# DefaultRui/VLN-VER

Measured on AMD Instinct MI355X. Metric: viewpoints/sec (multi-view->voxel fwd+bwd), vocc.py config, higher is better.
Workload: dtype bf16

## Files before the change

include/ver_ops.h:

```cpp
#ifndef VER_OPS_H
#define VER_OPS_H

#include <stdint.h>

#ifdef __cplusplus
extern "C" {
#endif

#define VER_ABI_VERSION 31

#define VER_OK            0
#define VER_EINVAL       -1
#define VER_EUNSUPPORTED -2
#define VER_ELAUNCH      -3

#define VER_F32  0
#define VER_BF16 1

int         ver_abi_version(void);
const char* ver_last_error(void);

int ver_msda_forward(const float* value, const int64_t* shapes_hw, const int64_t* level_start,
                     const float* loc, const float* attn_w, float* out,
                     int B, int num_keys, int heads, int head_dim, int levels, int points,
// ... 25 lines not shown

int ver_hits_from_mask(const uint8_t* bev_mask, int B, int Ncam, int Nq, int D,
                       uint8_t* vis, int32_t* vis_list, int32_t* vis_cnt,
                       int32_t* zero_list, int32_t* zero_cnt, int32_t* fwd_list, int32_t* fwd_cnt,
                       void* stream);

#define VER_SCA_ROWS_PREZEROED 1
#define VER_SCA_VALUE_HEAD_MAJOR 2
#define VER_SCA_GRAD_SLOTS_BF16 4
int ver_sca_head_major_supported(int value_dtype, int head_dim, int points, int map_h, int map_w);
int ver_sca_zero_rows(const int32_t* zero_list, const int32_t* zero_cnt, float* slots, int B, int Nq, int row_floats,
                      void* stream);
int ver_sca_forward(const void* value, int value_dtype, const float* offsets, const float* logits,
                    const float* uv, const uint8_t* vis, const int32_t* vis_list,
                    const int32_t* vis_cnt, const int32_t* zero_list, const int32_t* zero_cnt,
                    const int32_t* fwd_list, const int32_t* fwd_cnt,
                    float* slots,
                    int B, int Ncam, int Nq, int D, int heads, int head_dim, int points,
                    int map_h, int map_w, int flags, void* stream);

int ver_sca_backward_grad_dtype(int value_dtype, int head_dim, int points, int map_h, int map_w);
int ver_sca_backward(const void* value, int value_dtype, const float* offsets, const float* logits,
                     const float* uv, const uint8_t* vis, const int32_t* vis_list,
                     const int32_t* vis_cnt, const int32_t* fwd_list, const int32_t* fwd_cnt,
                     const void* grad_slots,
                     void* grad_value, int grad_value_dtype, float* grad_offsets, float* grad_logits,
                     int B, int Ncam, int Nq, int D, int heads, int head_dim, int points,
                     int map_h, int map_w, int flags, void* stream);

int ver_lattice_im2col(const void* src, void* col, const int* taps, int ntaps,
                       int B, int Z, int H, int W, int C, int dtype, void* stream);
int ver_lattice_col2im(const void* grad_col, void* grad_src, const int* taps, int ntaps,
                       int B, int Z, int H, int W, int C, int dtype, void* stream);

int ver_lattice_gather(const void* src, void* col, const int* taps, const long* col_offset, long col_stride,
                       int ntaps, int B, int Zr, int Zs, int H, int W, int C, int layout, int dtype,
                       const void* const_rows, const long* const_offset, int const_blocks, int const_width, void* stream);
int ver_lattice_scatter(const void* grad_col, void* grad_src, const int* taps, const long* col_offset,
                        long col_stride, int ntaps, int B, int Zr, int Zs, int H, int W, int C, int layout, int dtype,
                        void* stream);

int ver_convt_weight_forward(const float* weight, void* taps, long pairs, int dtype, void* stream);
int ver_convt_weight_backward(const void* grad_taps, float* grad_weight, long pairs, int dtype, void* stream);
int ver_convt_weight_backward_blocks(const void* blocks, const long* block_offsets, long ld, const void* prev_bias,
                                     const void* grad_v, float* grad_weight, int ci, int co, int dtype, void* stream);
int ver_convt_weight_forward_blocks(const float* weight, const long* block_offsets, long ld, void* blocks, int ci, int co,
                                    int dtype, void* stream);
int ver_blocks_vec_forward(const void* blocks, const long* block_rows, int nblocks, long ld, int ci, int ncols, const float* x,
                           float* vec, int dtype, void* stream);
int ver_blocks_vec_backward(const void* blocks, const long* block_rows, int nblocks, long ld, int ci, int ncols,
                            const float* grad_vec, float* grad_x, int dtype, void* stream);
int ver_lattice_transpose(void* channels_last, void* channel_first, long cf_stride, int B, int Z, int H, int W,
                          int C, int layout, int to_channel_first, int dtype, void* stream);
int ver_lattice_rows(void* channels_last, void* rows, long quarter, int period, int nseg, const int* seg_off,
                     const int* seg_len, const long* seg_base, const int* seg_pitch, const int* seg_rows, int B, int Z,
                     int H, int W, int C, int layout, int to_rows, int dtype, void* stream);

int ver_ln_relu_forward(const void* x, const float* gamma, const float* beta, void* y,
                        float* mean, float* rstd, long N, int W, float eps, int dtype, void* stream);
int ver_ln_relu_backward(const void* x, const void* grad_y, const float* gamma, const float* beta,
                         const float* mean, const float* rstd, void* grad_x,
                         float* grad_gamma, float* grad_beta, long N, int W, int dtype, void* stream);

int ver_focal_loss_blocks(long N, int C);
int ver_focal_loss_forward(const void* logits, const int64_t* target, float* partial, long N, int C,
                           float gamma, float alpha, int dtype, int32_t* bad_labels, void* stream);
int ver_focal_loss_forward_grad(const void* logits, const int64_t* target, float* partial, void* grad, long N, int C,
                                float gamma, float alpha, int dtype, int32_t* bad_labels, void* stream);
int ver_focal_loss_forward_grad_u8(const void* logits, const uint8_t* target, float* partial, void* grad, long N, int C,
                                   float gamma, float alpha, int dtype, int32_t* bad_labels, void* stream);
int ver_focal_loss_backward(const void* logits, const int64_t* target, const float* scale, void* grad,
                            long N, int C, float gamma, float alpha, int dtype, void* stream);

int ver_add_ln_forward(const void* a, int a_dtype, const float* residual, const float* gamma, const float* beta,
                       const int64_t* seed, float p_drop, float eps, float* y, void* y_bf16, float* mean,
                       float* rstd, long N, int C, void* stream);
int ver_add_ln_backward(const float* grad_y, const void* grad_y_bf16, const void* a, int a_dtype,
                        const float* residual, const float* gamma, const float* mean, const float* rstd,
                        const int64_t* seed, float p_drop, void* grad_a, float* grad_residual, float* grad_gamma,
                        float* grad_beta, long N, int C, void* stream);
int ver_relu_dropout_forward(const void* x, void* y, const int64_t* seed, float p_drop, long n, int dtype, void* stream);
int ver_relu_dropout_backward(const void* y, const void* grad_y, void* grad_x, float p_drop, long n, int dtype,
                              void* stream);

int ver_run_gather(const void* image, long image_stride, const int32_t* run_start, const int32_t* aug_idx,
                   void* rows, int B, int n_rows, int runs, int run_len, int n_aug, int row_elems, int dtype,
                   void* stream);
int ver_run_scatter(const void* rows, void* image, long image_stride, const int32_t* run_start, int B,
                    int n_rows, int runs, int run_len, int row_elems, int dtype, void* stream);

#define VER_OCC_MLP_CENTERED 2
long ver_occ_mlp_image_bytes(void);
int ver_occ_mlp_vector_floats(void);
int ver_occ_mlp_pack(const float* W1, const float* W2, const float* W3, void* image, void* stream);
int ver_occ_mlp_forward(const void* x, const void* image, const float* vectors, void* logits,
                        long N, int width, int classes, float eps, int first_linear, void* stream);
int ver_occ_mlp_forward_stats(const void* x, const void* image, const float* vectors, void* logits, float* rstd,
                              long N, int width, int classes, float eps, int first_linear, void* stream);
int ver_occ_mlp_backward(const void* x, const void* grad_logits, const void* image, const float* vectors,
                         void* grad_x, void* grad_a1, void* grad_a2, void* h1,
                         float* param_grads, long N, int width, int classes, float eps, int first_linear,
                         void* stream);
int ver_occ_mlp_backward_fused(const void* x, const void* grad_logits, const float* W2, const float* W3,
                               const float* vectors, void* grad_x, float* param_grads, long N, int width,
                               int classes, float eps, const float* grad_scale, int flags, void* stream);
int ver_occ_mlp_backward_fused_stats(const void* x, const void* grad_logits, const float* W2, const float* W3,
                                     const float* vectors, const float* rstd, void* grad_x, float* param_grads, long N,
                                     int width, int classes, float eps, const float* grad_scale, int flags, void* stream);

long ver_occ_predict_blocks(long N);
int  ver_occ_predict(const void* logits, int dtype, long N, int C, float threshold, int32_t* block_work,
                     int64_t* pairs, int64_t* count, void* stream);

int  ver_occ_confusion(const void* logits, int dtype, long rows_per_sample, int samples, int C, const uint8_t* labels,
                       const float* thresholds, int num_thresholds, int64_t* hist, void* stream);

int  ver_wgrad_tn_splits(long M, int Ka, int N);
int  ver_wgrad_tn_splits_ld(long M, int Ka, int N, long ld);
long ver_wgrad_tn_workspace(long M, int Ka, int N, int splits);
int  ver_wgrad_tn(const void* a, long lda, const void* g, long ldg, long M, int Ka, int N, void* out, long ldo,
                  int out_dtype, int splits, int flags, void* workspace, long workspace_bytes, void* stream);
int  ver_wgrad_tn_segments(const void* lattice, int layout, int B, int H, int W, int C, const int* taps, int nseg, const void* cst,
                           int ncst, int cw, const void* g, long ldg, int N, void* out, long ldo, int out_dtype, int splits,
                           void* workspace, long workspace_bytes, void* stream);
int  ver_wgrad_tn_segments_splits(int B, int H, int W, long Ka, int N, long ldg);

int  ver_gemm_nn(const void* a, long lda, const void* w, long ldw, const float* bias, void* c, long ldc, long M, int K,
                 int N, int flags, void* stream);
int  ver_gemm_nn_taps(const void* lattice, int layout, int B, int H, int W, int C, const int* taps, int ntaps, const void* w,
                      long ldw, const float* rowpos, const float* bias, void* c, long ldc, int N, void* stream);
int  ver_gemm_nn_segments(const void* lattice, int layout, int B, int H, int W, int C, const int* taps, int ntaps,
                          const void* cst, int ncst, int cw, const void* w, long ldw, const float* rowpos, const float* bias,
                          void* c, long ldc, int N, void* stream);
int  ver_gemm_nn_planes(const void* lattice, int layout, int B, int H, int W, int C, long plane_elems, int nplanes,
                        const int* tap_plane, const int* taps, int ntaps, const void* cst, int ncst, int cw, const void* w,
                        long ldw, const float* rowpos, const float* bias, void* c, long ldc, int N, void* stream);
int  ver_gemm_nn_splits(long M, int K, int N);
int  ver_gemm_nn_splitk(const void* a, long lda, const void* w, long ldw, const float* bias, void* c, long ldc, long M, int K,
                        int N, int splits, void* workspace, long workspace_bytes, void* stream);

int ver_clip_adamw_step(void* const* table, const long* sizes, const int* chunk_tensor, const int* chunk_index,
                        int n_tensors, int n_chunks, int chunk_elems, float* partial, float* norm_out, float max_norm,
                        float lr, float beta1, float beta2, float eps, float weight_decay, long step, void* stream);

int ver_clip_adamw_step_tensors(void* const* table, const long* sizes, const int* chunk_tensor, const int* chunk_index,
                                const float* hyper, int* steps, int n_tensors, int n_chunks, int chunk_elems, float* partial,
                                float* norm_out, float max_norm, void* stream);

int ver_lsa_solve(const float* cost, const int32_t* ncols, int32_t* match, int32_t* bad,
                  int P, int R, int Ccap, void* stream);

#ifdef __cplusplus
}
#endif
#endif
```

vln-ver_amd/csrc/ver_addln.hip:

```cpp
#include "ver_common.h"

namespace {
constexpr int kMaxK = 4;

__device__ __forceinline__ uint32_t f2bf(float f) {
    const uint32_t u = __float_as_uint(f);
    if ((u & 0x7fffffffu) > 0x7f800000u) return (u >> 16) | 0x40u;
    return (u + 0x7fffu + ((u >> 16) & 1u)) >> 16;
}

__device__ __forceinline__ bool keep_elem(uint64_t idx, uint64_t seed, uint32_t thresh) {
    uint64_t h = idx * 0x9E3779B97F4A7C15ull + seed;
    h ^= h >> 33;
    h *= 0xff51afd7ed558ccdull;
    h ^= h >> 33;
    h *= 0xc4ceb9fe1a85ec53ull;
    h ^= h >> 33;
    return (uint32_t)(h & 0xffffffu) < thresh;
}

template <bool ABF16>
__device__ __forceinline__ void load_a4(const void* a, long off, float (&v)[4]) {
    if (ABF16) {
        const uint2 t = *reinterpret_cast<const uint2*>(reinterpret_cast<const uint16_t*>(a) + off);
        v[0] = __uint_as_float(t.x << 16);
        v[1] = __uint_as_float(t.x & 0xffff0000u);
        v[2] = __uint_as_float(t.y << 16);
        v[3] = __uint_as_float(t.y & 0xffff0000u);
    } else {
        const float4 t = *reinterpret_cast<const float4*>(reinterpret_cast<const float*>(a) + off);
        v[0] = t.x; v[1] = t.y; v[2] = t.z; v[3] = t.w;
    }
}

__device__ __forceinline__ void store_bf4(uint16_t* p, long off, const float (&v)[4]) {
    uint2 t;
    t.x = f2bf(v[0]) | (f2bf(v[1]) << 16);
    t.y = f2bf(v[2]) | (f2bf(v[3]) << 16);
    *reinterpret_cast<uint2*>(p + off) = t;
}

template <bool ABF16, int K>
__device__ __forceinline__ void load_x(const void* a, const float* res, long row, int C, int lane, bool drop,
                                       uint64_t seed, uint32_t thresh, float scale, float (&x)[K][4],
                                       bool (&keep)[K][4]) {
#pragma unroll
    for (int k = 0; k < K; ++k) {
        const long off = row * C + 4 * (lane + 64 * k);
        float av[4];
        load_a4<ABF16>(a, off, av);
        const float4 r = *reinterpret_cast<const float4*>(res + off);
        const float rv[4] = {r.x, r.y, r.z, r.w};
#pragma unroll
        for (int i = 0; i < 4; ++i) {
            keep[k][i] = !drop || keep_elem((uint64_t)(off + i), seed, thresh);
            x[k][i] = rv[i] + (keep[k][i] ? av[i] * scale : 0.0f);
        }
    }
}
}

template <bool ABF16, int K>
__global__ __launch_bounds__(256) void k_add_ln_fwd(const void* __restrict__ a, const float* __restrict__ res,
                                                    const float* __restrict__ gamma, const float* __restrict__ beta,
                                                    const int64_t* __restrict__ seed_p, float p_drop, float eps,
                                                    float* __restrict__ y, uint16_t* __restrict__ y16,
                                                    float* __restrict__ mean, float* __restrict__ rstd, long N) {
    constexpr int C = 256 * K;
    const int lane = threadIdx.x & 63, wave = threadIdx.x >> 6;
    const bool drop = p_drop > 0.0f;
    const uint64_t seed = drop ? (uint64_t)seed_p[0] : 0ull;
    const uint32_t thresh = (uint32_t)((1.0f - p_drop) * 16777216.0f);
    const float scale = drop ? 1.0f / (1.0f - p_drop) : 1.0f;
    float g[K][4], bt[K][4];
#pragma unroll
    for (int k = 0; k < K; ++k) {
        const float4 gv = *reinterpret_cast<const float4*>(gamma + 4 * (lane + 64 * k));
        const float4 bv = *reinterpret_cast<const float4*>(beta + 4 * (lane + 64 * k));
        g[k][0] = gv.x; g[k][1] = gv.y; g[k][2] = gv.z; g[k][3] = gv.w;
        bt[k][0] = bv.x; bt[k][1] = bv.y; bt[k][2] = bv.z; bt[k][3] = bv.w;
    }
    for (long row = (long)blockIdx.x * 4 + wave; row < N; row += (long)gridDim.x * 4) {
        float x[K][4];
        bool keep[K][4];
        load_x<ABF16, K>(a, res, row, C, lane, drop, seed, thresh, scale, x, keep);
        float s = 0.0f;
#pragma unroll
        for (int k = 0; k < K; ++k) s += (x[k][0] + x[k][1]) + (x[k][2] + x[k][3]);
        const float mu = group_sum<64>(s) * (1.0f / C);
        float q = 0.0f;
#pragma unroll
        for (int k = 0; k < K; ++k)
#pragma unroll
            for (int i = 0; i < 4; ++i) {
                x[k][i] -= mu;
                q += x[k][i] * x[k][i];
            }
        const float rs = rsqrtf(group_sum<64>(q) * (1.0f / C) + eps);
        if (lane == 0) {
            mean[row] = mu;
            rstd[row] = rs;
        }
#pragma unroll
        for (int k = 0; k < K; ++k) {
            const long off = row * C + 4 * (lane + 64 * k);
            float o[4];
#pragma unroll
            for (int i = 0; i < 4; ++i) o[i] = x[k][i] * rs * g[k][i] + bt[k][i];
            *reinterpret_cast<float4*>(y + off) = make_float4(o[0], o[1], o[2], o[3]);
            if (y16) store_bf4(y16, off, o);
        }
    }
}

template <bool ABF16, int K>
__global__ __launch_bounds__(256) void k_add_ln_bwd(const float* __restrict__ dy, const uint16_t* __restrict__ dy16,
                                                    const void* __restrict__ a, const float* __restrict__ res,
                                                    const float* __restrict__ gamma, const float* __restrict__ mean,
                                                    const float* __restrict__ rstd, const int64_t* __restrict__ seed_p,
                                                    float p_drop, void* __restrict__ d_a, float* __restrict__ d_res,
                                                    float* __restrict__ dgamma, float* __restrict__ dbeta, long N) {
    constexpr int C = 256 * K;
    __shared__ float red[2][4][C];
    const int lane = threadIdx.x & 63, wave = threadIdx.x >> 6;
    const bool drop = p_drop > 0.0f;
    const uint64_t seed = drop ? (uint64_t)seed_p[0] : 0ull;
    const uint32_t thresh = (uint32_t)((1.0f - p_drop) * 16777216.0f);
    const float scale = drop ? 1.0f / (1.0f - p_drop) : 1.0f;
    float g[K][4], dg[K][4], db[K][4];
#pragma unroll
    for (int k = 0; k < K; ++k) {
        const float4 gv = *reinterpret_cast<const float4*>(gamma + 4 * (lane + 64 * k));
        g[k][0] = gv.x; g[k][1] = gv.y; g[k][2] = gv.z; g[k][3] = gv.w;
#pragma unroll
        for (int i = 0; i < 4; ++i) dg[k][i] = db[k][i] = 0.0f;
    }
    for (long row = (long)blockIdx.x * 4 + wave; row < N; row += (long)gridDim.x * 4) {
        float x[K][4], go[K][4];
        bool keep[K][4];
        load_x<ABF16, K>(a, res, row, C, lane, drop, seed, thresh, scale, x, keep);
        const float mu = mean[row], rs = rstd[row];
        float s1 = 0.0f, s2 = 0.0f;
#pragma unroll
        for (int k = 0; k < K; ++k) {
            const long off = row * C + 4 * (lane + 64 * k);
            const float4 t = *reinterpret_cast<const float4*>(dy + off);
            go[k][0] = t.x; go[k][1] = t.y; go[k][2] = t.z; go[k][3] = t.w;
            if (dy16) {
                float h[4];
                load_a4<true>(dy16, off, h);
#pragma unroll
                for (int i = 0; i < 4; ++i) go[k][i] += h[i];
            }
#pragma unroll
            for (int i = 0; i < 4; ++i) {
                x[k][i] = (x[k][i] - mu) * rs;
                dg[k][i] += go[k][i] * x[k][i];
                db[k][i] += go[k][i];
                go[k][i] *= g[k][i];
                s1 += go[k][i];
                s2 += go[k][i] * x[k][i];
            }
        }
        const float m1 = group_sum<64>(s1) * (1.0f / C), m2 = group_sum<64>(s2) * (1.0f / C);
#pragma unroll
        for (int k = 0; k < K; ++k) {
            const long off = row * C + 4 * (lane + 64 * k);
            float dx[4], da[4];
#pragma unroll
            for (int i = 0; i < 4; ++i) {
                dx[i] = (go[k][i] - m1 - x[k][i] * m2) * rs;
                da[i] = keep[k][i] ? dx[i] * scale : 0.0f;
            }
            *reinterpret_cast<float4*>(d_res + off) = make_float4(dx[0], dx[1], dx[2], dx[3]);
            if (ABF16)
                store_bf4(reinterpret_cast<uint16_t*>(d_a), off, da);
            else
                *reinterpret_cast<float4*>(reinterpret_cast<float*>(d_a) + off) = make_float4(da[0], da[1], da[2], da[3]);
        }
    }
#pragma unroll
    for (int k = 0; k < K; ++k)
#pragma unroll
        for (int i = 0; i < 4; ++i) {
            red[0][wave][4 * (lane + 64 * k) + i] = dg[k][i];
            red[1][wave][4 * (lane + 64 * k) + i] = db[k][i];
        }
    __syncthreads();
    for (int e = threadIdx.x; e < C; e += 256) {
        atomicAdd(dgamma + e, (red[0][0][e] + red[0][1][e]) + (red[0][2][e] + red[0][3][e]));
        atomicAdd(dbeta + e, (red[1][0][e] + red[1][1][e]) + (red[1][2][e] + red[1][3][e]));
    }
}

namespace {
int check_add_ln(const char* who, const void* a, const float* res, const float* gamma, long N, int C, int a_dtype,
                 float p_drop, const int64_t* seed) {
    VER_REQUIRE(N >= 0, VER_EINVAL, "%s: negative row count", who);
    VER_REQUIRE(C > 0 && C % 256 == 0 && C <= 256 * kMaxK, VER_EUNSUPPORTED,
                "%s: built for rows of 256, 512, 768 or 1024 channels (got %d)", who, C);
    VER_REQUIRE(a_dtype == VER_F32 || a_dtype == VER_BF16, VER_EINVAL, "%s: dtype %d is neither VER_F32 nor VER_BF16", who,
                a_dtype);
    VER_REQUIRE(p_drop >= 0.0f && p_drop < 1.0f, VER_EINVAL, "%s: dropout probability %g outside [0, 1)", who, p_drop);
    if (N == 0) return VER_OK;
    VER_REQUIRE(a && res && gamma && (seed || p_drop == 0.0f), VER_EINVAL, "%s: null pointer argument", who);
    VER_REQUIRE(((uintptr_t)a & 15) == 0 && ((uintptr_t)res & 15) == 0, VER_EINVAL, "%s: buffers must be 16-byte aligned", who);
    return VER_OK;
}
}

extern "C" int ver_add_ln_forward(const void* a, int a_dtype, const float* residual, const float* gamma,
                                  const float* beta, const int64_t* seed, float p_drop, float eps, float* y,
                                  void* y_bf16, float* mean, float* rstd, long N, int C, void* stream) {
    int rc = check_add_ln("ver_add_ln_forward", a, residual, gamma, N, C, a_dtype, p_drop, seed);
    if (rc) return rc;
    if (N == 0) return VER_OK;
    VER_REQUIRE(beta && y && mean && rstd, VER_EINVAL, "ver_add_ln_forward: null pointer argument");
    const unsigned grid = (unsigned)(((N + 3) / 4) < 8192 ? ((N + 3) / 4) : 8192);
    hipStream_t st = (hipStream_t)stream;
#define VER_FWD(BF, K_)                                                                                          \
    hipLaunchKernelGGL((k_add_ln_fwd<BF, K_>), dim3(grid), dim3(256), 0, st, a, residual, gamma, beta, seed, p_drop, \
                       eps, y, (uint16_t*)y_bf16, mean, rstd, N)
#define VER_FWD_K(BF)                        \
    do {                                     \
        if (C == 256) VER_FWD(BF, 1);        \
        else if (C == 512) VER_FWD(BF, 2);   \
        else if (C == 768) VER_FWD(BF, 3);   \
        else VER_FWD(BF, 4);                 \
    } while (0)
    if (a_dtype == VER_BF16) VER_FWD_K(true); else VER_FWD_K(false);
#undef VER_FWD_K
#undef VER_FWD
    return ver_check_launch("ver_add_ln_forward");
}

extern "C" int ver_add_ln_backward(const float* grad_y, const void* grad_y_bf16, const void* a, int a_dtype,
                                   const float* residual, const float* gamma, const float* mean, const float* rstd,
                                   const int64_t* seed, float p_drop, void* grad_a, float* grad_residual,
                                   float* grad_gamma, float* grad_beta, long N, int C, void* stream) {
    int rc = check_add_ln("ver_add_ln_backward", a, residual, gamma, N, C, a_dtype, p_drop, seed);
    if (rc) return rc;
    VER_REQUIRE(grad_gamma && grad_beta, VER_EINVAL, "ver_add_ln_backward: null parameter-gradient pointer");
    hipStream_t st = (hipStream_t)stream;
    int zrc = ver_zero_async(grad_gamma, C * sizeof(float), st);
    if (!zrc) zrc = ver_zero_async(grad_beta, C * sizeof(float), st);
    if (zrc) return zrc;
    hipError_t e = hipSuccess;
    if (e != hipSuccess) return ver_fail(VER_ELAUNCH, "ver_add_ln_backward: memset: %s", hipGetErrorString(e));
    if (N == 0) return VER_OK;
    VER_REQUIRE(grad_y && mean && rstd && grad_a && grad_residual, VER_EINVAL, "ver_add_ln_backward: null pointer argument");
    const unsigned grid = (unsigned)(((N + 3) / 4) < 2048 ? ((N + 3) / 4) : 2048);
#define VER_BWD(BF, K_)                                                                                           \
    hipLaunchKernelGGL((k_add_ln_bwd<BF, K_>), dim3(grid), dim3(256), 0, st, grad_y, (const uint16_t*)grad_y_bf16, a, \
                       residual, gamma, mean, rstd, seed, p_drop, grad_a, grad_residual, grad_gamma, grad_beta, N)
#define VER_BWD_K(BF)                        \
    do {                                     \
        if (C == 256) VER_BWD(BF, 1);        \
        else if (C == 512) VER_BWD(BF, 2);   \
        else if (C == 768) VER_BWD(BF, 3);   \
        else VER_BWD(BF, 4);                 \
    } while (0)
    if (a_dtype == VER_BF16) VER_BWD_K(true); else VER_BWD_K(false);
#undef VER_BWD_K
#undef VER_BWD
    return ver_check_launch("ver_add_ln_backward");
}

template <bool BF16>
__global__ __launch_bounds__(256) void k_relu_dropout_fwd(const void* __restrict__ x, void* __restrict__ y,
                                                          const int64_t* __restrict__ seed_p, float p_drop, long n4) {
    const bool drop = p_drop > 0.0f;
    const uint64_t seed = drop ? (uint64_t)seed_p[0] : 0ull;
    const uint32_t thresh = (uint32_t)((1.0f - p_drop) * 16777216.0f);
    const float scale = drop ? 1.0f / (1.0f - p_drop) : 1.0f;
    for (long i = (long)blockIdx.x * 256 + threadIdx.x; i < n4; i += (long)gridDim.x * 256) {
        float v[4];
        load_a4<BF16>(x, 4 * i, v);
#pragma unroll
        for (int j = 0; j < 4; ++j)
            v[j] = (v[j] > 0.0f && (!drop || keep_elem((uint64_t)(4 * i + j), seed, thresh))) ? v[j] * scale : 0.0f;
        if (BF16)
            store_bf4(reinterpret_cast<uint16_t*>(y), 4 * i, v);
        else
            *reinterpret_cast<float4*>(reinterpret_cast<float*>(y) + 4 * i) = make_float4(v[0], v[1], v[2], v[3]);
    }
}

template <bool BF16>
__global__ __launch_bounds__(256) void k_relu_dropout_bwd(const void* __restrict__ y, const void* __restrict__ dy,
                                                          void* __restrict__ dx, float scale, long n4) {
    for (long i = (long)blockIdx.x * 256 + threadIdx.x; i < n4; i += (long)gridDim.x * 256) {
        float v[4], g[4];
        load_a4<BF16>(y, 4 * i, v);
        load_a4<BF16>(dy, 4 * i, g);
#pragma unroll
        for (int j = 0; j < 4; ++j) g[j] = v[j] > 0.0f ? g[j] * scale : 0.0f;
        if (BF16)
            store_bf4(reinterpret_cast<uint16_t*>(dx), 4 * i, g);
        else
            *reinterpret_cast<float4*>(reinterpret_cast<float*>(dx) + 4 * i) = make_float4(g[0], g[1], g[2], g[3]);
    }
}

extern "C" int ver_relu_dropout_forward(const void* x, void* y, const int64_t* seed, float p_drop, long n, int dtype,
                                        void* stream) {
    VER_REQUIRE(n >= 0 && n % 4 == 0, VER_EINVAL, "ver_relu_dropout_forward: element count must be a multiple of 4");
    VER_REQUIRE(dtype == VER_F32 || dtype == VER_BF16, VER_EINVAL, "ver_relu_dropout_forward: dtype %d", dtype);
    VER_REQUIRE(p_drop >= 0.0f && p_drop < 1.0f, VER_EINVAL, "ver_relu_dropout_forward: dropout probability %g", p_drop);
    if (n == 0) return VER_OK;
    VER_REQUIRE(x && y && (seed || p_drop == 0.0f), VER_EINVAL, "ver_relu_dropout_forward: null pointer argument");
    const long n4 = n / 4;
    const unsigned grid = (unsigned)(((n4 + 255) / 256) < 16384 ? ((n4 + 255) / 256) : 16384);
    if (dtype == VER_BF16)
        hipLaunchKernelGGL(k_relu_dropout_fwd<true>, dim3(grid), dim3(256), 0, (hipStream_t)stream, x, y, seed, p_drop, n4);
    else
        hipLaunchKernelGGL(k_relu_dropout_fwd<false>, dim3(grid), dim3(256), 0, (hipStream_t)stream, x, y, seed, p_drop, n4);
    return ver_check_launch("ver_relu_dropout_forward");
}

extern "C" int ver_relu_dropout_backward(const void* y, const void* grad_y, void* grad_x, float p_drop, long n, int dtype,
                                         void* stream) {
    VER_REQUIRE(n >= 0 && n % 4 == 0, VER_EINVAL, "ver_relu_dropout_backward: element count must be a multiple of 4");
    VER_REQUIRE(dtype == VER_F32 || dtype == VER_BF16, VER_EINVAL, "ver_relu_dropout_backward: dtype %d", dtype);
    VER_REQUIRE(p_drop >= 0.0f && p_drop < 1.0f, VER_EINVAL, "ver_relu_dropout_backward: dropout probability %g", p_drop);
    if (n == 0) return VER_OK;
    VER_REQUIRE(y && grad_y && grad_x, VER_EINVAL, "ver_relu_dropout_backward: null pointer argument");
    const long n4 = n / 4;
    const unsigned grid = (unsigned)(((n4 + 255) / 256) < 16384 ? ((n4 + 255) / 256) : 16384);
    const float scale = 1.0f / (1.0f - p_drop);
    if (dtype == VER_BF16)
        hipLaunchKernelGGL(k_relu_dropout_bwd<true>, dim3(grid), dim3(256), 0, (hipStream_t)stream, y, grad_y, grad_x, scale, n4);
    else
        hipLaunchKernelGGL(k_relu_dropout_bwd<false>, dim3(grid), dim3(256), 0, (hipStream_t)stream, y, grad_y, grad_x, scale, n4);
    return ver_check_launch("ver_relu_dropout_backward");
}
```

vln-ver_amd/dense_heads/row_linear.py:

```python
import torch
import torch.nn.functional as F

_CHUNK = 8000


class _RowLinear(torch.autograd.Function):

    @staticmethod
    def forward(ctx, x, weight, bias):
        w = weight.to(x.dtype)
        ctx.save_for_backward(x, w)
        ctx.has_bias = bias is not None
        ctx.weight_dtype = weight.dtype
        if bias is None:
            return x @ w.t()
        return torch.addmm(bias.to(x.dtype), x, w.t())

    @staticmethod
    def backward(ctx, g):
        x, w = ctx.saved_tensors
        g = g.contiguous()
        n, o = g.shape
        gx = g @ w if ctx.needs_input_grad[0] else None
        gb = None
        if ctx.has_bias:
            gb = g.sum(0, dtype=torch.float32)
        if g.dtype == torch.bfloat16 and x.dtype == torch.bfloat16 and n >= 4096 and min(o, x.shape[1]) >= 192:
            from ..hipops import wgrad_tn, wgrad_tn_supported
            if wgrad_tn_supported(g, x):
                wide = torch.float32 if ctx.weight_dtype == torch.float32 else torch.bfloat16
                if wide == torch.bfloat16 and gb is not None:
                    gb = gb.to(torch.bfloat16)
                return gx, wgrad_tn(g, x, out_dtype=wide), gb
        s = n // _CHUNK
        main = s * _CHUNK
        gw = x.new_zeros((o, x.shape[1]), dtype=torch.float32)
        if s:
            g3 = g[:main].view(s, _CHUNK, o)
            gw += torch.bmm(g3.transpose(1, 2), x[:main].view(s, _CHUNK, -1)).sum(0, dtype=torch.float32)
        if main < n:
            gw += (g[main:].t() @ x[main:]).float()
        return gx, gw, gb


def row_linear(x, weight, bias):
    if not x.is_cuda:
        return F.linear(x, weight, bias)
    if torch.is_autocast_enabled('cuda'):
        x = x.to(torch.get_autocast_dtype('cuda'))
    shape = x.shape
    with torch.autocast('cuda', enabled=False):
        y = _RowLinear.apply(x.reshape(-1, shape[-1]), weight, bias)
    return y.view(*shape[:-1], -1)
```

vln-ver_amd/hipops.py:

```python
import ctypes
import os
import re

import torch
from torch.autograd import Function
from torch.autograd.function import once_differentiable

_PKG = os.path.dirname(os.path.abspath(__file__))
LIB_PATH = os.environ.get('VER_HIP_LIB') or os.path.join(_PKG, 'libver_hip.so')
ABI_VERSION = 31
HEADER = os.path.join(os.path.dirname(_PKG), 'include', 'ver_ops.h')
_PARAMS = {'int': ctypes.c_int, 'long': ctypes.c_long, 'float': ctypes.c_float}
_RETURNS = {'int': ctypes.c_int, 'long': ctypes.c_long, 'const char*': ctypes.c_char_p}


class HipLibraryError(RuntimeError):
    pass


def prototypes(path=HEADER):
    if not os.path.exists(path):
        raise HipLibraryError('%s not found: the C ABI is bound from its prototypes' % path)
    text = re.sub(r'/\*.*?\*/|//[^\n]*|^\s*#[^\n]*', ' ', open(path).read(), flags=re.S | re.M)
    out = {}
# ... 846 lines not shown
            vecs = pg[:768].view(6, 128)
            dw3 = pg[768:768 + 2048].view(16, 128)
            db3 = pg[768 + 2048:768 + 2048 + 16]
            dw2 = pg[768 + 2048 + 16:].view(128, 128)
            return (gx.view(shape), None, None, vecs[0], vecs[1], dw2, vecs[5], vecs[3], vecs[4], dw3, db3, None, None)
        gx, ga2, h1 = (torch.empty_like(x2) for _ in range(3))
        ga1 = None if ctx.folded else torch.empty_like(x2)
        pg = torch.empty(6 * 128 + 16 * 128 + 16, dtype=torch.float32, device=x.device)
        _launch('ver_occ_mlp_backward', lambda: lib().ver_occ_mlp_backward(
            _p(x2), _p(gl), _p(image), _p(vec), _p(gx), _p(ga1), _p(ga2), _p(h1), _p(pg),
            n, 128, 16, ctx.eps, 0 if ctx.folded else 1, _stream()))
        inv = _frag_order(x.device)
        vecs = pg[:768].view(6, 128)
        dw3 = pg[768:768 + 2048].view(16, 128)
        db3 = pg[768 + 2048:]
        dw2, _ = _rows_tn(ga2, h1, with_colsum=False)
        if ctx.folded:
            dw2 = dw2.index_select(0, inv)
            return (gx.view(shape), None, None, vecs[0], vecs[1], dw2, vecs[5], vecs[3], vecs[4], dw3, db3, None, None)
        dw2 = dw2.index_select(0, inv).index_select(1, inv)
        dw1, _ = _rows_tn(ga1, x2, with_colsum=False)
        dw1 = dw1.index_select(0, inv)
        return (gx.view(shape), dw1, vecs[2], vecs[0], vecs[1], dw2, vecs[5], vecs[3], vecs[4], dw3, db3, None, None)


class OccMLPFocalLossFunction(Function):

    @staticmethod
    def forward(ctx, x, g1, be1, w2, b2, g2, be2, w3, b3, target, eps, gamma, alpha, centered):
        x = _gpu(x, 'x').contiguous()
        image = occ_mlp_pack(w2, w2, w3)
        vec = occ_mlp_vectors(torch.zeros(128, device=x.device), g1, be1, b2, g2, be2, b3)
        ctx.has_rstd = _occ_mlp_wants_rstd(True, centered, x.numel() // 128)
        out = occ_mlp_forward(x, image, vec, eps, first_linear=False, centered=centered, want_rstd=ctx.has_rstd)
        logits, rstd = out if ctx.has_rstd else (out, None)
        l2 = logits.view(-1, 16)
        n = l2.shape[0]
        target = _gpu(target, 'target')
        as_bytes = target.dtype == torch.uint8
        target = (target if as_bytes else target.to(torch.int64)).contiguous()
        if target.shape != (n,):
            raise ValueError('target must be [N]')
        blocks = lib().ver_focal_loss_blocks(n, 16)
        partial = torch.zeros(blocks, dtype=torch.float32, device=x.device)
        flag = LabelRangeFlag.of(x.device)
        flag.poll()
        entry = lib().ver_focal_loss_forward_grad_u8 if as_bytes else lib().ver_focal_loss_forward_grad
        _launch('ver_focal_loss_forward_grad', lambda: entry(
            _p(l2), _p(target), _p(partial), _p(l2), n, 16, gamma, alpha, 1, _p(flag.dev), _stream()))
        flag.mirror(16)
        ctx.save_for_backward(x, vec, w2.detach(), w3.detach(), l2, *((rstd,) if ctx.has_rstd else ()))
        ctx.eps, ctx.centered = eps, bool(centered)
        return partial.sum()

    @staticmethod
    @once_differentiable
    def backward(ctx, grad_out):
        x, vec, w2, w3, gl = ctx.saved_tensors[:5]
        rstd = ctx.saved_tensors[5] if ctx.has_rstd else None
        shape = x.shape
        x2 = x.view(-1, 128)
        n = x2.shape[0]
        gscale = _gpu(grad_out, 'grad_out').float().reshape(1).contiguous()
        gx = torch.empty_like(x2)
        pg = torch.empty(6 * 128 + 16 * 128 + 16 + 128 * 128, dtype=torch.float32, device=x.device)
        _launch('ver_occ_mlp_backward_fused', lambda: lib().ver_occ_mlp_backward_fused_stats(
            _p(x2), _p(gl), _p(w2.float().contiguous()), _p(w3.float().contiguous()), _p(vec),
            _p(rstd), _p(gx), _p(pg), n, 128, 16, ctx.eps, _p(gscale), 2 if ctx.centered else 0, _stream()))
        vecs = pg[:768].view(6, 128)
        dw3 = pg[768:768 + 2048].view(16, 128)
        db3 = pg[768 + 2048:768 + 2048 + 16]
        dw2 = pg[768 + 2048 + 16:].view(128, 128)
        return (gx.view(shape), vecs[0], vecs[1], dw2, vecs[5], vecs[3], vecs[4], dw3, db3, None, None, None, None, None)


def occ_mlp_focal_loss_sum(x, g1, be1, w2, b2, g2, be2, w3, b3, target, eps=1e-5, gamma=2.0, alpha=0.25, centered=False):
    return OccMLPFocalLossFunction.apply(x, g1, be1, w2, b2, g2, be2, w3, b3, target, eps, float(gamma), float(alpha), centered)


def occ_mlp(x, w1, b1, g1, be1, w2, b2, g2, be2, w3, b3, eps=1e-5, centered=False):
    return OccMLPFunction.apply(x, w1, b1, g1, be1, w2, b2, g2, be2, w3, b3, eps, centered)


class AddDropoutLayerNormFunction(Function):

    @staticmethod
    def forward(ctx, a, residual, gamma, beta, p_drop, eps, want_bf16):
        a = _gpu(a, 'a')
        if a.dtype not in (torch.float32, torch.bfloat16):
            a = a.float()
        a = a.contiguous()
        res = _gpu(residual, 'residual').float().contiguous()
        C = a.shape[-1]
        n = a.numel() // C
        y = torch.empty_like(res)
        y16 = torch.empty(res.shape, dtype=torch.bfloat16, device=res.device) if want_bf16 else None
        mean = torch.empty(n, dtype=torch.float32, device=res.device)
        rstd = torch.empty_like(mean)
        seed = torch.randint(0, 2 ** 62, (1,), device=res.device, dtype=torch.int64) if p_drop > 0 else None
        g, b = gamma.detach().float().contiguous(), beta.detach().float().contiguous()
        _launch('ver_add_ln_forward', lambda: lib().ver_add_ln_forward(
            _p(a), 1 if a.dtype == torch.bfloat16 else 0, _p(res), _p(g), _p(b), _p(seed), p_drop, eps, _p(y), _p(y16),
            _p(mean), _p(rstd), n, C, _stream()))
        ctx.save_for_backward(a, res, g, mean, rstd, seed if seed is not None else torch.empty(0, device=res.device))
        ctx.p_drop, ctx.has_y16 = p_drop, want_bf16
        if want_bf16:
            return y, y16
        return y, None

    @staticmethod
    @once_differentiable
    def backward(ctx, grad_y, grad_y16):
        a, res, g, mean, rstd, seed = ctx.saved_tensors
        C = a.shape[-1]
        n = a.numel() // C
        gy = (torch.zeros_like(res) if grad_y is None else _gpu(grad_y, 'grad_y').float().contiguous())
        gy16 = None
        if ctx.has_y16 and grad_y16 is not None:
            gy16 = _gpu(grad_y16, 'grad_y_bf16').to(torch.bfloat16).contiguous()
        d_a = torch.empty_like(a)
        d_res = torch.empty_like(res)
        dg = torch.empty(C, dtype=torch.float32, device=res.device)
        db = torch.empty_like(dg)
        _launch('ver_add_ln_backward', lambda: lib().ver_add_ln_backward(
            _p(gy), _p(gy16), _p(a), 1 if a.dtype == torch.bfloat16 else 0, _p(res), _p(g), _p(mean), _p(rstd),
            _p(seed) if ctx.p_drop > 0 else None, ctx.p_drop, _p(d_a), _p(d_res), _p(dg), _p(db), n, C, _stream()))
        return d_a, d_res, dg, db, None, None, None


class ReluDropoutFunction(Function):

    @staticmethod
    def forward(ctx, x, p_drop):
        x = _gpu(x, 'x')
        if x.dtype not in (torch.float32, torch.bfloat16):
            x = x.float()
        x = x.contiguous()
        y = torch.empty_like(x)
        seed = torch.randint(0, 2 ** 62, (1,), device=x.device, dtype=torch.int64) if p_drop > 0 else None
        _launch('ver_relu_dropout_forward', lambda: lib().ver_relu_dropout_forward(
            _p(x), _p(y), _p(seed), p_drop, x.numel(), 1 if x.dtype == torch.bfloat16 else 0, _stream()))
        ctx.save_for_backward(y)
        ctx.p_drop = p_drop
        return y

    @staticmethod
    @once_differentiable
    def backward(ctx, grad_y):
        y, = ctx.saved_tensors
        gy = _gpu(grad_y, 'grad_y').to(y.dtype).contiguous()
        gx = torch.empty_like(y)
        _launch('ver_relu_dropout_backward', lambda: lib().ver_relu_dropout_backward(
            _p(y), _p(gy), _p(gx), ctx.p_drop, y.numel(), 1 if y.dtype == torch.bfloat16 else 0, _stream()))
        return gx, None


def relu_dropout(x, p_drop=0.0):
    return ReluDropoutFunction.apply(x, float(p_drop))


def add_dropout_layer_norm(a, residual, gamma, beta, p_drop=0.0, eps=1e-5, want_bf16=False):
    return AddDropoutLayerNormFunction.apply(a, residual, gamma, beta, float(p_drop), float(eps), bool(want_bf16))


class VoxelMSDeformAttnFunction(Function):

    @staticmethod
    def forward(ctx, value, spatial_shapes, level_start_index, sampling_locations, attention_weights):
        value = _gpu(value, 'value').float().contiguous()
        loc = _gpu(sampling_locations, 'sampling_locations').float().contiguous()
        aw = _gpu(attention_weights, 'attention_weights').float().contiguous()
        shapes = _gpu(spatial_shapes, 'spatial_shapes').to(torch.int64).contiguous()
        lsi = _gpu(level_start_index, 'level_start_index').to(torch.int64).contiguous()
        bs, nk, heads, hd = value.shape
        _, nq, _, nl, npt, _ = loc.shape
        out = value.new_empty(bs, nq, heads * hd)
        _launch('ver_msda3d_forward', lambda: lib().ver_msda3d_forward(
            _p(value), _p(shapes), _p(lsi), _p(loc), _p(aw), _p(out), bs, nk, heads, hd, nl, npt, nq, _stream()))
        ctx.save_for_backward(value, shapes, lsi, loc, aw)
        return out

    @staticmethod
    @once_differentiable
    def backward(ctx, grad_output):
        value, shapes, lsi, loc, aw = ctx.saved_tensors
        bs, nk, heads, hd = value.shape
        _, nq, _, nl, npt, _ = loc.shape
        gv, gl, ga = torch.zeros_like(value), torch.zeros_like(loc), torch.zeros_like(aw)
        go = _gpu(grad_output, 'grad_output').float().contiguous()
        _launch('ver_msda3d_backward', lambda: lib().ver_msda3d_backward(
            _p(value), _p(shapes), _p(lsi), _p(loc), _p(aw), _p(go), _p(gv), _p(gl), _p(ga), bs, nk, heads,
            hd, nl, npt, nq, _stream()))
        return gv, None, None, gl, ga


def voxel_msda(value, spatial_shapes, level_start_index, sampling_locations, attention_weights):
    return VoxelMSDeformAttnFunction.apply(value, spatial_shapes, level_start_index, sampling_locations,
                                           attention_weights)


def occ_predict(logits, threshold=0.25):
    logits = _gpu(logits, 'logits')
    if logits.dtype not in (torch.float32, torch.bfloat16):
        logits = logits.float()
    logits = logits.contiguous()
    n, c = logits.shape
    dt = 1 if logits.dtype == torch.bfloat16 else 0
    nb = lib().ver_occ_predict_blocks(n)
    work = torch.empty(max(nb, 1), dtype=torch.int32, device=logits.device)
    pairs = torch.empty(max(n, 1), 2, dtype=torch.int64, device=logits.device)
    count = torch.empty(1, dtype=torch.int64, device=logits.device)
    _launch('ver_occ_predict', lambda: lib().ver_occ_predict(
        _p(logits), dt, n, c, threshold, _p(work), _p(pairs), _p(count), _stream()))
    return pairs[:int(count.item())]


def occ_confusion(logits, labels, thresholds=(0.25,), samples=1, hist=None):
    logits = _gpu(logits, 'logits')
    if logits.dtype not in (torch.float32, torch.bfloat16):
        logits = logits.float()
    c = logits.shape[-1]
    logits = logits.reshape(-1, c).contiguous()
    labels = _gpu(labels, 'labels', torch.uint8).reshape(-1)
    n = logits.shape[0]
    if labels.numel() != n:
        raise ValueError('occ_confusion: %d labels for %d logit rows' % (labels.numel(), n))
    if samples < 1 or n % samples:
        raise ValueError('occ_confusion: %d rows do not split into %d samples' % (n, samples))
    thr = [float(t) for t in thresholds]
    k = c + 1
    shape = (samples, len(thr), k, k)
    if hist is None:
        hist = torch.zeros(shape, dtype=torch.int64, device=logits.device)
    elif (tuple(hist.shape) != shape or hist.dtype != torch.int64 or not hist.is_contiguous()
          or hist.device != logits.device):
        raise ValueError('occ_confusion: hist must be a contiguous int64 %s tensor on %s' % (shape, logits.device))
    dt = 1 if logits.dtype == torch.bfloat16 else 0
    host_thr = (ctypes.c_float * max(len(thr), 1))(*thr)
    _launch('ver_occ_confusion', lambda: lib().ver_occ_confusion(
        _p(logits), dt, n // samples, samples, c, _p(labels), host_thr, len(thr), _p(hist), _stream()))
    return hist


LSA_MAX = 1024

# ... 191 lines not shown
```

Before: 701.5.

## Fuse bias-gradient column sums into add-LN and ReLU-dropout backward kernels

The add-dropout-LayerNorm and ReLU-dropout backward kernels now also accumulate per-block column sums of the input gradient, and a small finishing kernel reduces them to the bias gradient. A side-channel box attached to the row_linear output passes this precomputed sum to the linear layer's backward, which then skips its separate g.sum(0) pass over the gradient. This saves a full read of the activation gradient per biased linear layer. In exchange it adds scratch buffers, a second small launch, per-row LDS read-modify-write traffic, and an occupancy hint on the K==3 add-LN kernel. It also relies on pointer identity to match the gradient, which is fragile.

```diff
diff --git a/include/ver_ops.h b/include/ver_ops.h
--- a/include/ver_ops.h
+++ b/include/ver_ops.h
@@ -131,6 +131,14 @@
 int ver_relu_dropout_forward(const void* x, void* y, const int64_t* seed, float p_drop, long n, int dtype, void* stream);
 int ver_relu_dropout_backward(const void* y, const void* grad_y, void* grad_x, float p_drop, long n, int dtype,
                               void* stream);
+long ver_add_ln_backward_colsum_scratch(long N, int C);
+int ver_add_ln_backward_colsum(const float* grad_y, const void* grad_y_bf16, const void* a, int a_dtype,
+                               const float* residual, const float* gamma, const float* mean, const float* rstd,
+                               const int64_t* seed, float p_drop, void* grad_a, float* grad_residual, float* grad_gamma,
+                               float* grad_beta, float* col_sum, float* col_scratch, long N, int C, void* stream);
+long ver_relu_dropout_backward_colsum_scratch(long N, int C);
+int ver_relu_dropout_backward_colsum(const void* y, const void* grad_y, void* grad_x, float p_drop, long N, int C, int dtype,
+                                     float* col_sum, float* col_scratch, void* stream);
 
 int ver_run_gather(const void* image, long image_stride, const int32_t* run_start, const int32_t* aug_idx,
                    void* rows, int B, int n_rows, int runs, int run_len, int n_aug, int row_elems, int dtype,
diff --git a/vln-ver_amd/csrc/ver_addln.hip b/vln-ver_amd/csrc/ver_addln.hip
--- a/vln-ver_amd/csrc/ver_addln.hip
+++ b/vln-ver_amd/csrc/ver_addln.hip
@@ -8,6 +8,8 @@
     if ((u & 0x7fffffffu) > 0x7f800000u) return (u >> 16) | 0x40u;
     return (u + 0x7fffu + ((u >> 16) & 1u)) >> 16;
 }
+
+__device__ __forceinline__ float bf_round(float f) { return __uint_as_float(f2bf(f) << 16); }
 
 __device__ __forceinline__ bool keep_elem(uint64_t idx, uint64_t seed, uint32_t thresh) {
     uint64_t h = idx * 0x9E3779B97F4A7C15ull + seed;
@@ -114,15 +116,17 @@
 }
 
 template <bool ABF16, int K>
-__global__ __launch_bounds__(256) void k_add_ln_bwd(const float* __restrict__ dy, const uint16_t* __restrict__ dy16,
+__global__ __launch_bounds__(256) __attribute__((amdgpu_waves_per_eu(K == 3 ? 4 : 1))) void k_add_ln_bwd(const float* __restrict__ dy, const uint16_t* __restrict__ dy16,
                                                     const void* __restrict__ a, const float* __restrict__ res,
                                                     const float* __restrict__ gamma, const float* __restrict__ mean,
                                                     const float* __restrict__ rstd, const int64_t* __restrict__ seed_p,
                                                     float p_drop, void* __restrict__ d_a, float* __restrict__ d_res,
-                                                    float* __restrict__ dgamma, float* __restrict__ dbeta, long N) {
+                                                    float* __restrict__ dgamma, float* __restrict__ dbeta,
+                                                    float* __restrict__ col_part, long N) {
     constexpr int C = 256 * K;
     __shared__ float red[2][4][C];
     const int lane = threadIdx.x & 63, wave = threadIdx.x >> 6;
+    const bool COLSUM = col_part != nullptr;
     const bool drop = p_drop > 0.0f;
     const uint64_t seed = drop ? (uint64_t)seed_p[0] : 0ull;
     const uint32_t thresh = (uint32_t)((1.0f - p_drop) * 16777216.0f);
@@ -134,6 +138,7 @@
         g[k][0] = gv.x; g[k][1] = gv.y; g[k][2] = gv.z; g[k][3] = gv.w;
 #pragma unroll
         for (int i = 0; i < 4; ++i) dg[k][i] = db[k][i] = 0.0f;
+        if (COLSUM) *reinterpret_cast<float4*>(&red[0][wave][4 * (lane + 64 * k)]) = make_float4(0.0f, 0.0f, 0.0f, 0.0f);
     }
     for (long row = (long)blockIdx.x * 4 + wave; row < N; row += (long)gridDim.x * 4) {
         float x[K][4], go[K][4];
@@ -172,6 +177,15 @@
                 dx[i] = (go[k][i] - m1 - x[k][i] * m2) * rs;
                 da[i] = keep[k][i] ? dx[i] * scale : 0.0f;
             }
+            if (COLSUM) {
+                float4* acc = reinterpret_cast<float4*>(&red[0][wave][4 * (lane + 64 * k)]);
+                float4 t = *acc;
+                t.x += ABF16 ? bf_round(da[0]) : da[0];
+                t.y += ABF16 ? bf_round(da[1]) : da[1];
+                t.z += ABF16 ? bf_round(da[2]) : da[2];
+                t.w += ABF16 ? bf_round(da[3]) : da[3];
+                *acc = t;
+            }
             *reinterpret_cast<float4*>(d_res + off) = make_float4(dx[0], dx[1], dx[2], dx[3]);
             if (ABF16)
                 store_bf4(reinterpret_cast<uint16_t*>(d_a), off, da);
@@ -179,6 +193,12 @@
                 *reinterpret_cast<float4*>(reinterpret_cast<float*>(d_a) + off) = make_float4(da[0], da[1], da[2], da[3]);
         }
     }
+    if (COLSUM) {
+        __syncthreads();
+        for (int e = threadIdx.x; e < C; e += 256)
+            col_part[(long)blockIdx.x * C + e] = (red[0][0][e] + red[0][1][e]) + (red[0][2][e] + red[0][3][e]);
+        __syncthreads();
+    }
 #pragma unroll
     for (int k = 0; k < K; ++k)
 #pragma unroll
@@ -190,6 +210,24 @@
     for (int e = threadIdx.x; e < C; e += 256) {
         atomicAdd(dgamma + e, (red[0][0][e] + red[0][1][e]) + (red[0][2][e] + red[0][3][e]));
         atomicAdd(dbeta + e, (red[1][0][e] + red[1][1][e]) + (red[1][2][e] + red[1][3][e]));
+    }
+}
+
+__global__ __launch_bounds__(1024) void k_col_sum_finish(const float* __restrict__ part, int nparts, int C,
+                                                         float* __restrict__ col_sum) {
+    __shared__ double red[32][33];
+    const int cx = threadIdx.x & 31, s = threadIdx.x >> 5;
+    const int c = blockIdx.x * 32 + cx;
+    double acc = 0.0;
+    if (c < C)
+        for (int p = s; p < nparts; p += 32) acc += (double)part[(long)p * C + c];
+    red[s][cx] = acc;
+    __syncthreads();
+    if (s == 0 && c < C) {
+        double t = 0.0;
+#pragma unroll
+        for (int j = 0; j < 32; ++j) t += red[j][cx];
+        col_sum[c] = (float)t;
     }
 }
 
@@ -234,25 +272,35 @@
     return ver_check_launch("ver_add_ln_forward");
 }
 
-extern "C" int ver_add_ln_backward(const float* grad_y, const void* grad_y_bf16, const void* a, int a_dtype,
-                                   const float* residual, const float* gamma, const float* mean, const float* rstd,
-                                   const int64_t* seed, float p_drop, void* grad_a, float* grad_residual,
-                                   float* grad_gamma, float* grad_beta, long N, int C, void* stream) {
-    int rc = check_add_ln("ver_add_ln_backward", a, residual, gamma, N, C, a_dtype, p_drop, seed);
+namespace {
+constexpr int kAddLnBwdBlocks = 2048, kReluBwdRowBlocks = 1024;
+unsigned add_ln_bwd_grid(long N) { return (unsigned)(((N + 3) / 4) < kAddLnBwdBlocks ? ((N + 3) / 4) : kAddLnBwdBlocks); }
+
+int launch_col_sum_finish(const char* who, const float* part, int nparts, int C, float* col_sum, hipStream_t st) {
+    hipLaunchKernelGGL(k_col_sum_finish, dim3((unsigned)((C + 31) / 32)), dim3(1024), 0, st, part, nparts, C, col_sum);
+    return ver_check_launch(who);
+}
+
+int add_ln_backward(const char* who, const float* grad_y, const void* grad_y_bf16, const void* a, int a_dtype,
+                    const float* residual, const float* gamma, const float* mean, const float* rstd, const int64_t* seed,
+                    float p_drop, void* grad_a, float* grad_residual, float* grad_gamma, float* grad_beta, float* col_sum,
+                    float* col_scratch, long N, int C, void* stream) {
+    int rc = check_add_ln(who, a, residual, gamma, N, C, a_dtype, p_drop, seed);
     if (rc) return rc;
-    VER_REQUIRE(grad_gamma && grad_beta, VER_EINVAL, "ver_add_ln_backward: null parameter-gradient pointer");
+    VER_REQUIRE(grad_gamma && grad_beta, VER_EINVAL, "%s: null parameter-gradient pointer", who);
     hipStream_t st = (hipStream_t)stream;
     int zrc = ver_zero_async(grad_gamma, C * sizeof(float), st);
     if (!zrc) zrc = ver_zero_async(grad_beta, C * sizeof(float), st);
+    if (!zrc && col_sum && N == 0) zrc = ver_zero_async(col_sum, C * sizeof(float), st);
     if (zrc) return zrc;
-    hipError_t e = hipSuccess;
-    if (e != hipSuccess) return ver_fail(VER_ELAUNCH, "ver_add_ln_backward: memset: %s", hipGetErrorString(e));
     if (N == 0) return VER_OK;
-    VER_REQUIRE(grad_y && mean && rstd && grad_a && grad_residual, VER_EINVAL, "ver_add_ln_backward: null pointer argument");
-    const unsigned grid = (unsigned)(((N + 3) / 4) < 2048 ? ((N + 3) / 4) : 2048);
+    VER_REQUIRE(grad_y && mean && rstd && grad_a && grad_residual, VER_EINVAL, "%s: null pointer argument", who);
+    VER_REQUIRE(!col_sum || col_scratch, VER_EINVAL, "%s: null pointer argument (col_scratch)", who);
+    const unsigned grid = add_ln_bwd_grid(N);
+    float* col_part = col_sum ? col_scratch : nullptr;
 #define VER_BWD(BF, K_)                                                                                           \
     hipLaunchKernelGGL((k_add_ln_bwd<BF, K_>), dim3(grid), dim3(256), 0, st, grad_y, (const uint16_t*)grad_y_bf16, a, \
-                       residual, gamma, mean, rstd, seed, p_drop, grad_a, grad_residual, grad_gamma, grad_beta, N)
+                       residual, gamma, mean, rstd, seed, p_drop, grad_a, grad_residual, grad_gamma, grad_beta, col_part, N)
 #define VER_BWD_K(BF)                        \
     do {                                     \
         if (C == 256) VER_BWD(BF, 1);        \
@@ -263,7 +311,32 @@
     if (a_dtype == VER_BF16) VER_BWD_K(true); else VER_BWD_K(false);
 #undef VER_BWD_K
 #undef VER_BWD
-    return ver_check_launch("ver_add_ln_backward");
+    rc = ver_check_launch(who);
+    if (rc || !col_sum) return rc;
+    return launch_col_sum_finish(who, col_scratch, (int)grid, C, col_sum, st);
+}
+}
+
+extern "C" int ver_add_ln_backward(const float* grad_y, const void* grad_y_bf16, const void* a, int a_dtype,
+                                   const float* residual, const float* gamma, const float* mean, const float* rstd,
+                                   const int64_t* seed, float p_drop, void* grad_a, float* grad_residual,
+                                   float* grad_gamma, float* grad_beta, long N, int C, void* stream) {
+    return add_ln_backward("ver_add_ln_backward", grad_y, grad_y_bf16, a, a_dtype, residual, gamma, mean, rstd, seed, p_drop,
+                           grad_a, grad_residual, grad_gamma, grad_beta, nullptr, nullptr, N, C, stream);
+}
+
+extern "C" long ver_add_ln_backward_colsum_scratch(long N, int C) {
+    if (N <= 0 || C <= 0 || C % 256 != 0 || C > 256 * kMaxK) return 0;
+    return (long)add_ln_bwd_grid(N) * C;
+}
+
+extern "C" int ver_add_ln_backward_colsum(const float* grad_y, const void* grad_y_bf16, const void* a, int a_dtype,
+                                          const float* residual, const float* gamma, const float* mean, const float* rstd,
+                                          const int64_t* seed, float p_drop, void* grad_a, float* grad_residual,
+                                          float* grad_gamma, float* grad_beta, float* col_sum, float* col_scratch, long N,
+                                          int C, void* stream) {
+    return add_ln_backward("ver_add_ln_backward_colsum", grad_y, grad_y_bf16, a, a_dtype, residual, gamma, mean, rstd, seed,
+                           p_drop, grad_a, grad_residual, grad_gamma, grad_beta, col_sum, col_scratch, N, C, stream);
 }
 
 template <bool BF16>
@@ -300,6 +373,31 @@
         else
             *reinterpret_cast<float4*>(reinterpret_cast<float*>(dx) + 4 * i) = make_float4(g[0], g[1], g[2], g[3]);
     }
+}
+
+template <bool BF16>
+__global__ __launch_bounds__(1024) void k_relu_dropout_bwd_rows(const void* __restrict__ y, const void* __restrict__ dy,
+                                                                void* __restrict__ dx, float scale, long N,
+                                                                float* __restrict__ col_part) {
+    const long c4 = blockDim.x;
+    float cs[4] = {0.0f, 0.0f, 0.0f, 0.0f};
+#pragma unroll 4
+    for (long row = blockIdx.x; row < N; row += gridDim.x) {
+        const long i = row * c4 + threadIdx.x;
+        float v[4], g[4];
+        load_a4<BF16>(y, 4 * i, v);
+        load_a4<BF16>(dy, 4 * i, g);
+#pragma unroll
+        for (int j = 0; j < 4; ++j) {
+            g[j] = v[j] > 0.0f ? g[j] * scale : 0.0f;
+            cs[j] += BF16 ? bf_round(g[j]) : g[j];
+        }
+        if (BF16)
+            store_bf4(reinterpret_cast<uint16_t*>(dx), 4 * i, g);
+        else
+            *reinterpret_cast<float4*>(reinterpret_cast<float*>(dx) + 4 * i) = make_float4(g[0], g[1], g[2], g[3]);
+    }
+    *reinterpret_cast<float4*>(col_part + ((long)blockIdx.x * c4 + threadIdx.x) * 4) = make_float4(cs[0], cs[1], cs[2], cs[3]);
 }
 
 extern "C" int ver_relu_dropout_forward(const void* x, void* y, const int64_t* seed, float p_drop, long n, int dtype,
@@ -334,3 +432,33 @@
         hipLaunchKernelGGL(k_relu_dropout_bwd<false>, dim3(grid), dim3(256), 0, (hipStream_t)stream, y, grad_y, grad_x, scale, n4);
     return ver_check_launch("ver_relu_dropout_backward");
 }
+
+extern "C" long ver_relu_dropout_backward_colsum_scratch(long N, int C) {
+    if (N <= 0 || C <= 0 || C % 256 != 0 || C > 4096) return 0;
+    return (N < kReluBwdRowBlocks ? N : kReluBwdRowBlocks) * C;
+}
+
+extern "C" int ver_relu_dropout_backward_colsum(const void* y, const void* grad_y, void* grad_x, float p_drop, long N, int C,
+                                                int dtype, float* col_sum, float* col_scratch, void* stream) {
+    VER_REQUIRE(N >= 0 && C > 0, VER_EINVAL, "ver_relu_dropout_backward_colsum: bad sizes");
+    if (!col_sum) return ver_relu_dropout_backward(y, grad_y, grad_x, p_drop, N * C, dtype, stream);
+    VER_REQUIRE(C % 256 == 0 && C <= 4096, VER_EUNSUPPORTED,
+                "ver_relu_dropout_backward_colsum: built for rows of a multiple of 256 up to 4096 channels (got %d)", C);
+    VER_REQUIRE(dtype == VER_F32 || dtype == VER_BF16, VER_EINVAL, "ver_relu_dropout_backward_colsum: dtype %d", dtype);
+    VER_REQUIRE(p_drop >= 0.0f && p_drop < 1.0f, VER_EINVAL, "ver_relu_dropout_backward_colsum: dropout probability %g", p_drop);
+    hipStream_t st = (hipStream_t)stream;
+    if (N == 0) return ver_zero_async(col_sum, C * sizeof(float), st);
+    VER_REQUIRE(y && grad_y && grad_x && col_scratch, VER_EINVAL, "ver_relu_dropout_backward_colsum: null pointer argument");
+    VER_REQUIRE(((uintptr_t)y & 15) == 0 && ((uintptr_t)grad_y & 15) == 0 && ((uintptr_t)grad_x & 15) == 0 &&
+                    ((uintptr_t)col_scratch & 15) == 0,
+                VER_EINVAL, "ver_relu_dropout_backward_colsum: buffers must be 16-byte aligned");
+    const unsigned grid = (unsigned)(N < kReluBwdRowBlocks ? N : kReluBwdRowBlocks);
+    const float scale = 1.0f / (1.0f - p_drop);
+    if (dtype == VER_BF16)
+        hipLaunchKernelGGL(k_relu_dropout_bwd_rows<true>, dim3(grid), dim3(C / 4), 0, st, y, grad_y, grad_x, scale, N, col_scratch);
+    else
+        hipLaunchKernelGGL(k_relu_dropout_bwd_rows<false>, dim3(grid), dim3(C / 4), 0, st, y, grad_y, grad_x, scale, N, col_scratch);
+    int rc = ver_check_launch("ver_relu_dropout_backward_colsum");
+    if (rc) return rc;
+    return launch_col_sum_finish("ver_relu_dropout_backward_colsum", col_scratch, (int)grid, C, col_sum, st);
+}
diff --git a/vln-ver_amd/dense_heads/row_linear.py b/vln-ver_amd/dense_heads/row_linear.py
--- a/vln-ver_amd/dense_heads/row_linear.py
+++ b/vln-ver_amd/dense_heads/row_linear.py
@@ -7,10 +7,11 @@
 class _RowLinear(torch.autograd.Function):
 
     @staticmethod
-    def forward(ctx, x, weight, bias):
+    def forward(ctx, x, weight, bias, box=None):
         w = weight.to(x.dtype)
         ctx.save_for_backward(x, w)
         ctx.has_bias = bias is not None
+        ctx.box = box
         ctx.weight_dtype = weight.dtype
         if bias is None:
             return x @ w.t()
@@ -24,14 +25,16 @@
         gx = g @ w if ctx.needs_input_grad[0] else None
         gb = None
         if ctx.has_bias:
-            gb = g.sum(0, dtype=torch.float32)
+            gb = ctx.box.take(g) if ctx.box is not None else None
+            if gb is None:
+                gb = g.sum(0, dtype=torch.float32)
         if g.dtype == torch.bfloat16 and x.dtype == torch.bfloat16 and n >= 4096 and min(o, x.shape[1]) >= 192:
             from ..hipops import wgrad_tn, wgrad_tn_supported
             if wgrad_tn_supported(g, x):
                 wide = torch.float32 if ctx.weight_dtype == torch.float32 else torch.bfloat16
                 if wide == torch.bfloat16 and gb is not None:
                     gb = gb.to(torch.bfloat16)
-                return gx, wgrad_tn(g, x, out_dtype=wide), gb
+                return gx, wgrad_tn(g, x, out_dtype=wide), gb, None
         s = n // _CHUNK
         main = s * _CHUNK
         gw = x.new_zeros((o, x.shape[1]), dtype=torch.float32)
@@ -40,7 +43,7 @@
             gw += torch.bmm(g3.transpose(1, 2), x[:main].view(s, _CHUNK, -1)).sum(0, dtype=torch.float32)
         if main < n:
             gw += (g[main:].t() @ x[main:]).float()
-        return gx, gw, gb
+        return gx, gw, gb, None
 
 
 def row_linear(x, weight, bias):
@@ -49,6 +52,13 @@
     if torch.is_autocast_enabled('cuda'):
         x = x.to(torch.get_autocast_dtype('cuda'))
     shape = x.shape
+    box = None
+    if bias is not None:
+        from ..hipops import BiasGradBox
+        box = BiasGradBox()
     with torch.autocast('cuda', enabled=False):
-        y = _RowLinear.apply(x.reshape(-1, shape[-1]), weight, bias)
-    return y.view(*shape[:-1], -1)
+        y = _RowLinear.apply(x.reshape(-1, shape[-1]), weight, bias, box)
+    y = y.view(*shape[:-1], -1)
+    if box is not None:
+        y._ver_bias_grad_box = box
+    return y
diff --git a/vln-ver_amd/hipops.py b/vln-ver_amd/hipops.py
--- a/vln-ver_amd/hipops.py
+++ b/vln-ver_amd/hipops.py
@@ -952,10 +952,35 @@
     return OccMLPFunction.apply(x, w1, b1, g1, be1, w2, b2, g2, be2, w3, b3, eps, centered)
 
 
+class BiasGradBox:
+    __slots__ = ('grad', 'col_sum')
+
+    def __init__(self):
+        self.grad = self.col_sum = None
+
+    def put(self, grad, col_sum):
+        self.grad, self.col_sum = grad, col_sum
+
+    def take(self, g):
+        grad, col_sum = self.grad, self.col_sum
+        self.grad = self.col_sum = None
+        if (grad is not None and g.data_ptr() == grad.data_ptr() and g.numel() == grad.numel() and g.dtype == grad.dtype
+                and g.is_contiguous() and g.shape[-1] == col_sum.numel()):
+            return col_sum
+        return None
+
+
+def _col_sum_buffers(scratch_floats, width, device):
+    if scratch_floats <= 0:
+        return None, None
+    return (torch.empty(width, dtype=torch.float32, device=device),
+            torch.empty(scratch_floats, dtype=torch.float32, device=device))
+
+
 class AddDropoutLayerNormFunction(Function):
 
     @staticmethod
-    def forward(ctx, a, residual, gamma, beta, p_drop, eps, want_bf16):
+    def forward(ctx, a, residual, gamma, beta, p_drop, eps, want_bf16, box=None):
         a = _gpu(a, 'a')
         if a.dtype not in (torch.float32, torch.bfloat16):
             a = a.float()
@@ -973,7 +998,7 @@
             _p(a), 1 if a.dtype == torch.bfloat16 else 0, _p(res), _p(g), _p(b), _p(seed), p_drop, eps, _p(y), _p(y16),
             _p(mean), _p(rstd), n, C, _stream()))
         ctx.save_for_backward(a, res, g, mean, rstd, seed if seed is not None else torch.empty(0, device=res.device))
-        ctx.p_drop, ctx.has_y16 = p_drop, want_bf16
+        ctx.p_drop, ctx.has_y16, ctx.box = p_drop, want_bf16, box
         if want_bf16:
             return y, y16
         return y, None
@@ -992,16 +1017,21 @@
         d_res = torch.empty_like(res)
         dg = torch.empty(C, dtype=torch.float32, device=res.device)
         db = torch.empty_like(dg)
-        _launch('ver_add_ln_backward', lambda: lib().ver_add_ln_backward(
+        cs, scratch = (None, None) if ctx.box is None else _col_sum_buffers(
+            lib().ver_add_ln_backward_colsum_scratch(n, C), C, res.device)
+        _launch('ver_add_ln_backward', lambda: lib().ver_add_ln_backward_colsum(
             _p(gy), _p(gy16), _p(a), 1 if a.dtype == torch.bfloat16 else 0, _p(res), _p(g), _p(mean), _p(rstd),
-            _p(seed) if ctx.p_drop > 0 else None, ctx.p_drop, _p(d_a), _p(d_res), _p(dg), _p(db), n, C, _stream()))
-        return d_a, d_res, dg, db, None, None, None
+            _p(seed) if ctx.p_drop > 0 else None, ctx.p_drop, _p(d_a), _p(d_res), _p(dg), _p(db), _p(cs), _p(scratch), n, C,
+            _stream()))
+        if cs is not None:
+            ctx.box.put(d_a, cs)
+        return d_a, d_res, dg, db, None, None, None, None
 
 
 class ReluDropoutFunction(Function):
 
     @staticmethod
-    def forward(ctx, x, p_drop):
+    def forward(ctx, x, p_drop, box=None):
         x = _gpu(x, 'x')
         if x.dtype not in (torch.float32, torch.bfloat16):
             x = x.float()
@@ -1011,7 +1041,7 @@
         _launch('ver_relu_dropout_forward', lambda: lib().ver_relu_dropout_forward(
             _p(x), _p(y), _p(seed), p_drop, x.numel(), 1 if x.dtype == torch.bfloat16 else 0, _stream()))
         ctx.save_for_backward(y)
-        ctx.p_drop = p_drop
+        ctx.p_drop, ctx.box = p_drop, box
         return y
 
     @staticmethod
@@ -1020,17 +1050,28 @@
         y, = ctx.saved_tensors
         gy = _gpu(grad_y, 'grad_y').to(y.dtype).contiguous()
         gx = torch.empty_like(y)
-        _launch('ver_relu_dropout_backward', lambda: lib().ver_relu_dropout_backward(
-            _p(y), _p(gy), _p(gx), ctx.p_drop, y.numel(), 1 if y.dtype == torch.bfloat16 else 0, _stream()))
-        return gx, None
+        C = y.shape[-1] if y.dim() else 1
+        n = y.numel() // max(C, 1)
+        cs, scratch = (None, None) if ctx.box is None else _col_sum_buffers(
+            lib().ver_relu_dropout_backward_colsum_scratch(n, C), C, y.device)
+        if cs is None:
+            _launch('ver_relu_dropout_backward', lambda: lib().ver_relu_dropout_backward(
+                _p(y), _p(gy), _p(gx), ctx.p_drop, y.numel(), 1 if y.dtype == torch.bfloat16 else 0, _stream()))
+        else:
+            _launch('ver_relu_dropout_backward', lambda: lib().ver_relu_dropout_backward_colsum(
+                _p(y), _p(gy), _p(gx), ctx.p_drop, n, C, 1 if y.dtype == torch.bfloat16 else 0, _p(cs), _p(scratch),
+                _stream()))
+            ctx.box.put(gx, cs)
+        return gx, None, None
 
 
 def relu_dropout(x, p_drop=0.0):
-    return ReluDropoutFunction.apply(x, float(p_drop))
+    return ReluDropoutFunction.apply(x, float(p_drop), getattr(x, '_ver_bias_grad_box', None))
 
 
 def add_dropout_layer_norm(a, residual, gamma, beta, p_drop=0.0, eps=1e-5, want_bf16=False):
-    return AddDropoutLayerNormFunction.apply(a, residual, gamma, beta, float(p_drop), float(eps), bool(want_bf16))
+    return AddDropoutLayerNormFunction.apply(a, residual, gamma, beta, float(p_drop), float(eps), bool(want_bf16),
+                                             getattr(a, '_ver_bias_grad_box', None))
 
 
 class VoxelMSDeformAttnFunction(Function):
```

Measured after the change: 703.1, median of 6. No clear change (+0.2%).
